# google-research/tnco

Hardware: AMD Instinct MI355X
Metric: SA move-evaluations/s (whole node) + best log10(flops) vs ref, 512-leaf TN (higher is better)
Workload: dtype f64

## Files before the change

tnco_amd/csrc/sa_sweep.h:

```cpp
#pragma once
#include "sa_kernels.h"
#include "fw_params.h"

#include <type_traits>

namespace tnco {

#define TNCO_LANDED(x) __asm__ volatile("" : "+v"(x) : : "memory")

#ifndef TNCO_NODE_ACCESS
#define TNCO_NODE_ACCESS 4
#endif

#define TNCO_LDS __attribute__((address_space(3)))
typedef TNCO_LDS volatile uint32_t lds_vu32;
typedef TNCO_LDS volatile int32_t lds_vi32;

__device__ __forceinline__ uint32_t mt_temper(uint32_t z) {
  z ^= (z >> 11);
  z ^= (z << 7) & 0x9d2c5680u;
  z ^= (z << 15) & 0xefc60000u;
  z ^= (z >> 18);
  return z;
}

constexpr int MT_SHADOW = 64;

constexpr int MT_ROUND_RING = 64;
constexpr int MT_ROUND_LOW = 8;
static_assert(MT_ROUND_RING <= MT_SHADOW && MT_ROUND_LOW >= 7, "refill rounds");

typedef uint32_t rng_u32x4 __attribute__((ext_vector_type(4)));
struct RngPcv { rng_u32x4 pcv; };
struct RngNoPcv {};
template <int LOG2L, int RINGX = 0, bool PCV = false>
struct Rng : std::conditional_t<PCV, RngPcv, RngNoPcv> {
  static constexpr int L = 1 << LOG2L;
  static constexpr int NL = L < 4 ? L : 4;
  static constexpr int SB = 4 * NL;
  static constexpr int RING = RINGX ? RINGX : ((2 * SB > 16) ? 2 * SB : 16);
  static_assert(RING <= MT_SHADOW && (RING & (RING - 1)) == 0 && RING >= 2 * SB, "ring size");

  struct __attribute__((packed, aligned(4))) U4 { uint32_t x[4]; };

  uint32_t* mt_base;
  uint32_t* sh_base;
  uint32_t r32;
  lds_vu32* ring;
  int lig;
  __device__ __forceinline__ uint32_t* st() const { return mt_base + (uint64_t)r32 * 624u; }
  __device__ __forceinline__ uint32_t* shadow() const { return sh_base + (uint64_t)r32 * (uint32_t)MT_SHADOW; }
  uint32_t cons, prod, tw;
  bool pend, ptw;
  typedef rng_u32x4 u32x4;
  u32x4 pa;
  uint32_t pb, pc[4];
  typedef u32x4 u32x4w __attribute__((aligned(4)));

  __device__ __forceinline__ uint32_t gen_of_cons() const { return cons == 0 ? 0u : (cons - 1u) / 624u; }

  __device__ __forceinline__ void request() {
    const uint32_t k0 = prod % 624u;
    ptw = prod >= tw;
    if (lig < NL) {
      const int k = (int)k0 + 4 * lig;
      const uint32_t* s = st();
      pa = *reinterpret_cast<const u32x4*>(s + k);
      if (ptw) {
        pb = s[(k + 4 == 624) ? 0 : k + 4];
        if (k == 224) {
          if constexpr (PCV) { this->pcv.x = s[621]; this->pcv.y = s[622]; this->pcv.z = s[623]; this->pcv.w = s[0]; }
          else { pc[0] = s[621]; pc[1] = s[622]; pc[2] = s[623]; pc[3] = s[0]; }
        } else {
          int km = k + 397;
          if (km >= 624) km -= 624;
          if constexpr (PCV) {
            this->pcv = *reinterpret_cast<const u32x4w*>(s + km);
          } else {
            const U4 c = *reinterpret_cast<const U4*>(s + km);
            pc[0] = c.x[0]; pc[1] = c.x[1]; pc[2] = c.x[2]; pc[3] = c.x[3];
          }
        }
      }
    }
    pend = true;
  }
  __device__ __forceinline__ void produce() {
    if (lig < NL) {
      const uint32_t nx[4] = {pa[1], pa[2], pa[3], pb};
      uint32_t v[4];
#pragma unroll
      for (int j = 0; j < 4; ++j) {
        v[j] = pa[j];
        if (ptw) {
          const uint32_t y = (pa[j] & 0x80000000u) | (nx[j] & 0x7fffffffu);
          uint32_t c;
          if constexpr (PCV) c = this->pcv[j]; else c = pc[j];
          v[j] = c ^ (y >> 1) ^ ((y & 1u) ? 0x9908b0dfu : 0u);
        }
        ring[(prod + (uint32_t)(4 * lig + j)) & (RING - 1)] = mt_temper(v[j]);
      }
      if (ptw) {
        const int sidx = (int)(prod % 624u) + 4 * lig;
        *reinterpret_cast<uint4*>(st() + sidx) = make_uint4(v[0], v[1], v[2], v[3]);
        if ((prod / 624u) > gen_of_cons())
          *reinterpret_cast<uint4*>(shadow() + sidx) = make_uint4(pa[0], pa[1], pa[2], pa[3]);
      }
    }
    if (ptw) tw = prod + SB;
    prod += SB;
    pend = false;
  }
  __device__ __forceinline__ bool room() const { return !pend && (prod - cons) + SB <= (uint32_t)RING; }

  template <int FILL = 0>
  __device__ __forceinline__ void init(const Params& P, int64_t r, lds_vu32* ring_, int mti, int mtw,
                                       int lig_) {
    mt_base = P.mt; sh_base = P.mtshadow; r32 = (uint32_t)r; ring = ring_; lig = lig_;
    pend = false; ptw = false;
    pb = 0;
    pa = (u32x4)(0u);
#pragma unroll
    for (int j = 0; j < 4; ++j) pc[j] = 0;
    if constexpr (PCV) this->pcv = (u32x4)(0u);
    if (mti >= 624) { cons = 624; tw = 624; } else { cons = (uint32_t)mti; tw = (uint32_t)mtw; }
    prod = cons & ~(uint32_t)(SB - 1);
    for (int b = 0; (FILL == 0 || b < FILL) && room(); ++b) {
      request();
      produce();
    }
  }
  __device__ __forceinline__ uint32_t next() {
    const uint32_t v = ring[cons & (RING - 1)];
    ++cons;
    return v;
  }
  __device__ __forceinline__ uint32_t next_sync() {
    if (cons == prod) {
      if (!pend) request();
      produce();
    }
    return next();
  }
  __device__ __forceinline__ void prefetch() {
    if (room()) request();
  }
  __device__ __forceinline__ uint32_t avail() const { return prod - cons; }
  __device__ __forceinline__ double uniform01() {
    const uint32_t x1 = next();
    const uint32_t x2 = next();
    double s = (double)x1 + (double)x2 * 4294967296.0;
    double r = s * 5.421010862427522170037e-20;
    if (r >= 1.0) r = 0.99999999999999988897769753748;
    return r;
  }
  __device__ __forceinline__ void finish(int& mti, int& mtw) {
    if (pend) produce();
    const uint32_t g = gen_of_cons();
    mti = (int)(cons - 624u * g);
    if (tw > 624u * (g + 1u)) {
      const uint32_t nw = tw - 624u * (g + 1u);
      for (uint32_t k = (uint32_t)lig; k < nw; k += L) st()[k] = shadow()[k];
      mtw = 624;
    } else {
      mtw = (int)(tw - 624u * g);
    }
  }
};

#ifndef TNCO_ACCEPT_PATH
#define TNCO_ACCEPT_PATH(p)
#endif

__device__ __attribute__((noinline)) bool accept_exact(double x, double beta, double u, int f32) {
  return u <= rnd_cost(pow(x, -beta), f32);
}

__device__ __forceinline__ bool accept_move(int kind, double beta, double delta, double total, double u,
                                            int f32) {
  if (kind == 0) { TNCO_ACCEPT_PATH(0); return true; }
  if (delta <= 0) { TNCO_ACCEPT_PATH(0); return true; }
  if (kind == 1) { TNCO_ACCEPT_PATH(1); return u <= 0.0; }
  if (total == 0) { TNCO_ACCEPT_PATH(1); return u <= 0.0; }
  const double x = rnd_cost(1.0 + rnd_cost(delta / total, f32), f32);
  const float uf = (float)u, xf = (float)x, bf = (float)beta;
  const float lu = __log2f(uf), lx = __log2f(xf);
  const float lp = -bf * lx;
  const float margin = (fabsf(lp) + fabsf(lu)) * 2e-6f + fabsf(bf) * 3e-7f + 1e-5f;
  if (uf > 1e-30f && xf < 1e30f && fabsf(lp) < 1e30f && beta >= 0.0) {
#ifdef TNCO_CHECK_ACCEPT
    if (lu < lp - margin || lu > lp + margin) {
      const bool fast = lu < lp - margin;
      if (fast != accept_exact(x, beta, u, f32)) __builtin_trap();
      return fast;
    }
#else
    if (lu < lp - margin) { TNCO_ACCEPT_PATH(2); return true; }
    if (lu > lp + margin) { TNCO_ACCEPT_PATH(3); return false; }
#endif
  }
  TNCO_ACCEPT_PATH(4);
  return accept_exact(x, beta, u, f32);
}

#ifndef TNCO_WAVES_PER_SIMD
#define TNCO_WAVES_PER_SIMD 3
#endif
enum : int { S_BEGIN = 0, S_GOT_B = 1, S_GOT_HB = 2, S_GOT_B1 = 3, S_GOT_HA = 4, S_MOVE = 5, S_END = 6 };

struct WalkScal {
  double total, beta, pP, pO, pC, raC, rnC;
  int raL, raR, raP, rnL, rnR, rnP, raW, rnW;
  uint32_t n_moves, n_acc;
};
struct ColdState {
  double min_cost;
  uint32_t jmin, n_impr, n_full, n_rpick;
};
typedef TNCO_LDS volatile ColdState lds_cold;

#ifdef TNCO_PROFILE
#define TNCO_PROF_DECL unsigned long long pt_[5] = {0, 0, 0, 0, 0}, pa_[5] = {0, 0, 0, 0, 0}
#if TNCO_PROFILE == 2
#define TNCO_PROF_T(i)                                           \
  do {                                                           \
    if ((i) == 1) pt_[0] = __builtin_amdgcn_s_memtime();         \
    if ((i) == 2) pt_[4] = __builtin_amdgcn_s_memtime();         \
  } while (0)
#define TNCO_PROF_F(i) pt_[i] = __builtin_amdgcn_s_memtime()
#else
#define TNCO_PROF_T(i) pt_[i] = __builtin_amdgcn_s_memtime()
#define TNCO_PROF_F(i)
#endif
#define TNCO_PROF_ACC                                            \
  do {                                                           \
    pa_[0] += pt_[1] - pt_[0]; pa_[1] += pt_[2] - pt_[1];        \
    pa_[2] += pt_[3] - pt_[2]; pa_[3] += pt_[4] - pt_[3];        \
    pa_[4] += 1;                                                 \
  } while (0)
#define TNCO_PROF_OUT(rs) \
  for (int k_ = 0; k_ < 5; ++k_) (rs)->pad1[k_] += pa_[k_]
#else
#define TNCO_PROF_DECL
#define TNCO_PROF_T(i)
#define TNCO_PROF_F(i)
#define TNCO_PROF_ACC
#define TNCO_PROF_OUT(rs)
#endif

#ifndef TNCO_SWEEP_THREADS
#define TNCO_SWEEP_THREADS 256
#endif
constexpr int SWT = TNCO_SWEEP_THREADS;
#ifndef TNCO_FW_STAGED_WAVES
#define TNCO_FW_STAGED_WAVES 2
#endif
#ifndef TNCO_LEAN_RULE
#define TNCO_LEAN_RULE (FW && !GENERIC && !HYPER && LOG2L == 2)
#endif
template <int LOG2L, int K, bool HYPER, bool GENERIC, bool FW = false, bool SPREAD = false>
#ifndef TNCO_HYPER_WAVES
#define TNCO_HYPER_WAVES 2
#endif
#ifndef TNCO_GENERIC_WAVES
#define TNCO_GENERIC_WAVES 2
#endif
#ifndef TNCO_K4_WAVES
#define TNCO_K4_WAVES 2
#endif
__device__ __forceinline__ void sa_run_body(
    const Params& P, const double* __restrict__ betas, const int64_t n_steps, const int prob_kind,
    const FwParams& F, const int tail_last, const int block0) {
  constexpr int L = 1 << LOG2L;
  constexpr int GPB = SWT >> LOG2L;
  using M = Mask<K>;
  constexpr bool ROUNDS = !HYPER && !GENERIC && !FW;
  constexpr bool RPCV = ROUNDS && TNCO_NODE_ACCESS >= 4;
  using R = Rng<LOG2L, ROUNDS ? MT_ROUND_RING : 0, RPCV>;
  static_assert(!ROUNDS || R::SB + 1 >= MT_ROUND_LOW, "refill rounds: the prologue");
  __shared__ uint32_t rngbuf[GPB * R::RING];
  __shared__ ColdState coldbuf[GPB];
  __shared__ int32_t jbuf[GPB * 16];
  constexpr bool LEAN = TNCO_LEAN_RULE;
  __shared__ WalkScal scalbuf[LEAN ? GPB : 1];
  __shared__ uint64_t slbuf[LEAN && FW ? GPB * L * K : 1];
  __shared__ double tabbuf[GENERIC ? (L * K * 64 + 1) : 1];
  __shared__ uint64_t clsbuf[GENERIC ? (TABS_MAXCLS * L * K) : 1];
  __shared__ uint64_t oddbuf[GENERIC ? (L * K) : 1];
  if constexpr (GENERIC) {
    const bool use_ctab = P.cost_mode == 1 || (P.cost_mode == 2 && P.odd_single);
    if (use_ctab) {
      for (int i = threadIdx.x; i < P.W * 64 + 1; i += SWT) tabbuf[i] = P.ctab[i];
    } else if (P.cost_mode == 2) {
      for (int i = threadIdx.x; i < L * K * 64; i += SWT) tabbuf[i] = P.dimsd[i];
    }
    if (P.cost_mode >= 2) {
      for (int i = threadIdx.x; i < P.n_dimclass * L * K; i += SWT) clsbuf[i] = P.dimclass[i];
      if (P.cost_mode == 2)
        for (int i = threadIdx.x; i < L * K; i += SWT) oddbuf[i] = P.oddmask[i];
    }
    __syncthreads();
  }

  const int tid = threadIdx.x;
  const int lig = tid & (L - 1);
  const int gbase = (tid & 63) & ~(L - 1);
  const int seats = SPREAD ? block0 : (64 >> LOG2L);
  const int gw = (tid & 63) >> LOG2L;
  const bool master = !SPREAD || gw < seats;
  const int seat = SPREAD ? (gw & (seats - 1)) : gw;
  const int gib = SPREAD ? (tid >> 6) * (64 >> LOG2L) + seat : tid >> LOG2L;
  const int64_t r = SPREAD ? ((int64_t)blockIdx.x * (SWT / 64) + (tid >> 6)) * seats + seat
                           : ((int64_t)blockIdx.x + block0) * GPB + gib;
  if (r >= P.R || n_steps <= 0) return;
  const bool lane0 = (lig == 0) && master;
  const int slig = master ? lig : (1 << 20);

  const int n = P.n, N = P.N;
  constexpr bool HYD = HYPER;
  constexpr bool CP = !HYPER && !GENERIC && !FW;
  constexpr bool QHDR = CP && TNCO_NODE_ACCESS >= 1, PAIRS = CP && TNCO_NODE_ACCESS >= 2, PSEL = CP && TNCO_NODE_ACCESS >= 3 && LPS == 1;
  View<LOG2L, K, HYPER, !FW, PAIRS> v;
  v.init(P, P.blocks + r * P.RB, nullptr, lig);
  auto lpar = [&]() -> int32_t* { return P.lpar + r * (int64_t)n * LPS; };
  lds_cold& cold = *((lds_cold*)coldbuf + gib);

  R rng;
  {
    const ReplicaState* rs = P.rs + r;
    rng.template init<ROUNDS ? 2 : 0>(P, r, (lds_vu32*)rngbuf + gib * R::RING, rs->mti, rs->mtw, master ? lig : 64);
    if (lane0) {
      cold.min_cost = rs->min_cost;
      cold.jmin = rs->jmin;
      cold.n_impr = 0; cold.n_full = 0; cold.n_rpick = 0;
    }
  }
  const uint32_t jcap = (uint32_t)P.jcap;
  uint32_t jtail = P.rs[r].jtail;
  bool jinvalid = P.rs[r].jinvalid != 0;
  auto jb = [&](int i) -> lds_vi32& { return *((lds_vi32*)jbuf + gib * 16 + i); };
  auto jlog = [&]() -> int32_t* {
    uint32_t rr = rng.r32;
    __asm__ volatile("" : "+v"(rr));
    return P.jlog + (int64_t)rr * (int64_t)P.jcap;
  };
  if ((jtail & 15u) != 0u) {
    for (int q = slig; q < 4; q += L) {
      const int4 t = *reinterpret_cast<const int4*>(jlog() + (jtail & ~15u) + 4 * q);
      jb(4 * q + 0) = t.x; jb(4 * q + 1) = t.y; jb(4 * q + 2) = t.z; jb(4 * q + 3) = t.w;
    }
  }
  M sl_regs = mzero<K>();
  typedef TNCO_LDS volatile uint64_t lds_vu64;
  [[maybe_unused]] lds_vu64* slw = (lds_vu64*)slbuf + (LEAN && FW ? gib * (L * K) : 0);
  [[maybe_unused]] bool impr_any = false;
  if constexpr (FW) {
    const uint64_t* s0 = F.slices + r * 2 * (int64_t)(L * K);
#pragma unroll
    for (int k = 0; k < K; ++k) {
      if constexpr (LEAN && FW) slw[v.widx(k)] = s0[v.widx(k)]; else sl_regs.w[k] = s0[v.widx(k)];
    }
  }
  [[maybe_unused]] TabsLds<K> tabs{P, (lds_cdouble*)tabbuf, (lds_cu64*)clsbuf, (lds_cu64*)oddbuf, mzero<K>()};
  if constexpr (GENERIC) {
    if (P.sparse != nullptr) {
#pragma unroll
      for (int k = 0; k < K; ++k) tabs.sp.w[k] = P.sparse[k * L + lig];
    }
  }
  const int f32 = GENERIC ? P.f32 : 0;
  const int log2d = P.log2d;
  const bool disable_shared = P.disable_shared != 0;
  const int nsteps32 = (int)n_steps;

  int B = 0, bl = 0, br = 0, A = -1;
  [[maybe_unused]] int wB = 0;
  double ccB = 0, partB = 0;
  WalkScal scal_regs{0, 0, 0, 0, 0, 0, 0, -1, -1, -1, -1, -1, -1, 0, 0, 0, 0};
  TNCO_LDS volatile WalkScal* scal_lds = (TNCO_LDS volatile WalkScal*)scalbuf + (LEAN ? gib : 0);
  auto& S = *[&]() {
    if constexpr (LEAN) return scal_lds; else return &scal_regs;
  }();
  if constexpr (CP) {
    double t0 = P.rs[r].total;
    TNCO_LANDED(t0);
    S.total = t0;
  }
  if constexpr (LEAN) {
    S.total = 0; S.beta = 0; S.pP = 0; S.pO = 0; S.pC = 0; S.raC = 0; S.rnC = 0;
    S.raL = -1; S.raR = -1; S.raP = -1; S.rnL = -1; S.rnR = -1; S.rnP = -1; S.raW = 0; S.rnW = 0; S.n_moves = 0; S.n_acc = 0;
  }
  M mP = mzero<K>(), mO = mzero<K>(), hB = mzero<K>();
  bool pl = true;
  M mC = mzero<K>(), hA = mzero<K>();
  int step = 0;
  int state = S_BEGIN;

  int stC = 0, stE = 0;
  [[maybe_unused]] double stW64 = 0;
  [[maybe_unused]] double stQ0 = 0, stQ1 = 0;
  int x_al = 0, x_ar = 0, x_aP = -1;
  double x_ccA = 0, x_partA = 0, x_pCcur = 0;
  int gL = -1, gR = -1, gP = -1;
  [[maybe_unused]] int gW = 0;
  double gC = 0;
  [[maybe_unused]] double gQ1 = 0;
  typedef int32_t i32x4 __attribute__((ext_vector_type(4)));
  [[maybe_unused]] i32x4 gLRP = (i32x4)(-1);
  [[maybe_unused]] u32x2 gHq = (u32x2)(0u);
  M gM = mzero<K>(), gH = mzero<K>();
  [[maybe_unused]] PairStage<K> gMq;
  if constexpr (PAIRS) {
#pragma unroll
    for (int j = 0; j < (K / 2 ? K / 2 : 1); ++j) gMq.p[j] = (u64x2)(0ull);
    gMq.s = 0ull;
  }
  uint32_t gXlo = 0, gXhi = 0;

  TNCO_PROF_DECL;
  for (;;) {
    TNCO_PROF_T(0);
    if (rng.pend) rng.produce();
    TNCO_PROF_T(1);

    bool acc = false, did_move = false, did_end = false, improved = false;

    if (state == S_END) {
      did_end = true;
      const bool close_sweep = !FW || tail_last != 0 || step != nsteps32 - 1;
      if constexpr (CP) {
        stQ0 = pl ? S.pP : S.pO;
        stQ1 = pl ? S.pO : S.pP;
      }
      if (close_sweep && partB < cold.min_cost) {
        if constexpr (FW) impr_any = true;
        if (lane0) {
          cold.min_cost = partB;
          cold.n_impr = cold.n_impr + 1;
        }
        if (jinvalid) {
          if (lane0) {
            NodeRec o;
            o.left = bl; o.right = br; o.parent = -1; o.pad = 0; o.ccost = CP ? stQ0 : ccB; o.partial = CP ? stQ1 : partB;
            *v.hdr(B) = o;
          }
          v.lpar = lpar();
          Links* __restrict__ ml = P.minlinks + r * (int64_t)N;
          for (int i0 = slig; i0 < N; i0 += 4 * L) {
            int4 h4[4];
#pragma unroll
            for (int q = 0; q < 4; ++q) {
              const int i = i0 + q * L;
              h4[q] = make_int4(-1, -1, -1, 0);
              if (i < n) h4[q].z = v.lpar[(int64_t)i * LPS];
              else if (i < N) h4[q] = *reinterpret_cast<const int4*>(v.hdr(i));
            }
#pragma unroll
            for (int q = 0; q < 4; ++q) {
              const int i = i0 + q * L;
              if (i < N) {
                Links o;
                o.left = h4[q].x; o.right = h4[q].y; o.parent = h4[q].z; o.pad = 0;
                ml[i] = o;
              }
            }
          }
          jtail = 0;
          jinvalid = false;
          if (lane0) cold.n_full = cold.n_full + 1;
        }
        improved = true;
      }
      if constexpr (CP) S.total = partB;
      ++step;
      state = (step >= nsteps32) ? -1 : S_BEGIN;
    }

    TNCO_PROF_F(1);
    int hN = -1, x1 = -1, yN = -1;
    const uint32_t* xa = nullptr;
    if (state == S_BEGIN) {
      const uint32_t x = rng.next();
      x_al = (int)(x % (uint32_t)n);
      x1 = x_al;
      xa = reinterpret_cast<const uint32_t*>(lpar() + (int64_t)x_al * LPS);
    } else if (state == S_GOT_B) {
      hN = B;
      if constexpr (CP) x1 = B;
      else xa = reinterpret_cast<const uint32_t*>(&v.hdr(B)->partial);
    } else if (CP && state == S_GOT_HB) {
      xa = reinterpret_cast<const uint32_t*>(betas + step);
      if (A >= 0) {
        hN = A;
        x1 = A;
      }
    } else if (state == S_GOT_HB) {
      x1 = pl ? br : bl;
      hN = A;
      yN = B;
      xa = reinterpret_cast<const uint32_t*>(&v.hdr(N - 1)->partial);
    } else if (state == S_GOT_B1) {
      xa = reinterpret_cast<const uint32_t*>(betas + step);
      if (A >= 0) {
        hN = S.raP;
        yN = A;
        x1 = (S.raL == B) ? S.raR : S.raL;
      }
    } else if (state == S_MOVE) {
      if constexpr (CP) {
        if (S.raP >= 0) {
          hN = S.raP;
          x1 = S.raP;
        }
      } else if (S.raP >= 0) {
        x1 = (S.rnL == A) ? S.rnR : S.rnL;
        hN = S.rnP;
        yN = S.raP;
      }
    }

    TNCO_PROF_F(2);
    if constexpr (QHDR) {
      int lq = lig;
      __asm__ volatile("" : "+v"(lq));
      v.lig = lq;
    }
    if (hN >= 0) {
      const NodeRec* q = v.hdr(hN);
      if constexpr (QHDR) {
        gHq = *reinterpret_cast<const u32x2*>(v.blk + v.hdr_piece_off(hN));
      } else {
        if constexpr (CP) gLRP = *reinterpret_cast<const i32x4*>(q);
        else { gL = q->left; gR = q->right; gP = q->parent; }
        gC = q->ccost;
        if constexpr (FW) gW = q->pad;
        if constexpr (CP) gQ1 = q->pright;
      }
    }
    double gMp = 0;
    if (x1 >= 0) {
      if constexpr (PAIRS) v.pair_stage_into(gMq, x1);
      else v.mask_stage_into(gM, x1);
      if constexpr (!CP)
        if (x1 >= n) gMp = v.hdr(x1)->partial;
    }
    if (xa != nullptr) {
      gXlo = xa[0];
      gXhi = xa[1];
    }
    if constexpr (HYPER) {
      if (yN >= 0) v.mask_stage_into(gH, yN);
    }
    if constexpr (ROUNDS) {
      const bool need = !rng.pend && rng.avail() < (uint32_t)MT_ROUND_LOW;
      const bool round = __ballot(need) != 0;
      if (round && rng.room()) rng.request();
    } else {
      if (rng.room()) rng.request();
    }
    TNCO_PROF_F(3);

    if (state == S_MOVE) {
      did_move = true;
      int al = S.raL, ar = S.raR;
      const int aP = S.raP;
      double ccA = S.raC;
      const bool c_is_right = (al == B);
      const int C = c_is_right ? ar : al;

      const M hy = HYD ? mand<K>(hB, mor<K>(mand<K>(hA, mC), mand<K>(mP, mO))) : mzero<K>();
      M sl = sl_regs;
      if constexpr (LEAN && FW) {
#pragma unroll
        for (int k = 0; k < K; ++k) sl.w[k] = slw[v.widx(k)];
      }
      constexpr bool PICK_FIRST = !GENERIC && FW;
      bool interP, interO;
      int pcAP = 0, pcBP = 0, pcAO = 0, pcBO = 0;
      if constexpr (!GENERIC && !PICK_FIRST) {
        uint32_t wP = mpopc<K>(mor<K>(mor<K>(mor<K>(mxor<K>(mP, mC), hy), mO), sl)) |
                      (mpopc<K>(mor<K>(mor<K>(mP, mC), sl)) << 13) | ((mnonzero<K>(mand<K>(mP, mC)) ? 1u : 0u) << 26);
        uint32_t wO = mpopc<K>(mor<K>(mor<K>(mor<K>(mxor<K>(mO, mC), hy), mP), sl)) |
                      (mpopc<K>(mor<K>(mor<K>(mO, mC), sl)) << 13) | ((mnonzero<K>(mand<K>(mO, mC)) ? 1u : 0u) << 26);
        wP = gsum<LOG2L>(wP);
        wO = gsum<LOG2L>(wO);
        interP = (wP >> 26) != 0;
        interO = (wO >> 26) != 0;
        pcAP = (int)(wP & 0x1fffu); pcBP = (int)((wP >> 13) & 0x1fffu);
        pcAO = (int)(wO & 0x1fffu); pcBO = (int)((wO >> 13) & 0x1fffu);
      } else {
        const uint32_t w = gsum<LOG2L>((mnonzero<K>(mand<K>(mP, mC)) ? 1u : 0u) |
                                       ((mnonzero<K>(mand<K>(mO, mC)) ? 1u : 0u) << 8));
        interP = (w & 0xffu) != 0;
        interO = (w >> 8) != 0;
      }
      bool pick0;
      if (disable_shared || (interP && interO)) {
        pick0 = (rng.next() & 1u) != 0;
        if (lane0) cold.n_rpick = cold.n_rpick + 1;
      } else {
        pick0 = pl ? interP : interO;
      }
      const bool pickP = pick0 == pl;
      const M mD = msel<K>(pickP, mP, mO), mE = msel<K>(pickP, mO, mP);
      const M newB = mor<K>(mxor<K>(mD, mC), hy);
      const double pD = pickP ? S.pP : S.pO, pE = pickP ? S.pO : S.pP;
      const int E = pick0 ? br : bl;
      if constexpr (PICK_FIRST) {
        const uint32_t w = gsum<LOG2L>(mpopc<K>(mor<K>(mor<K>(newB, mE), sl)) | (mpopc<K>(mor<K>(mor<K>(mD, mC), sl)) << 13));
        pcAP = pcAO = (int)(w & 0x1fffu);
        pcBP = pcBO = (int)((w >> 13) & 0x1fffu);
      }

      [[maybe_unused]] double new_width_B = 0;
      bool fits = true;
      if constexpr (FW) {
        double sliced_width;
        if constexpr (!GENERIC) {
          const uint32_t x = gsum<LOG2L>(mpopc<K>(newB) | (mpopc<K>(mandn<K>(newB, sl)) << 16));
          new_width_B = (double)(log2d * (int)(x & 0xffffu));
          sliced_width = (double)(log2d * (int)(x >> 16));
        } else if (F.log2dims == nullptr && P.sparse == nullptr) {
          const uint32_t x = gsum<LOG2L>(mpopc<K>(newB) | (mpopc<K>(mandn<K>(newB, sl)) << 16));
          new_width_B = fw_wr(F, F.log2d * (double)(x & 0xffffu));
          sliced_width = fw_wr(F, F.log2d * (double)(x >> 16));
        } else {
          new_width_B = fw_width<LOG2L, K>(P, F, newB, lig, gbase);
          sliced_width = fw_width<LOG2L, K>(P, F, mandn<K>(newB, sl), lig, gbase);
        }
        fits = sliced_width <= F.max_width;
      }
      double nA, nB;
      if constexpr (!GENERIC) {
        nA = pow2_cost(log2d * (pickP ? pcAP : pcAO), 0);
        nB = pow2_cost(log2d * (pickP ? pcBP : pcBO), 0);
      } else {
        nA = generic_cost_t<LOG2L, K>(P, tabs, mor<K>(mor<K>(newB, mE), sl), lig, gbase);
        nB = generic_cost_t<LOG2L, K>(P, tabs, mor<K>(mor<K>(mD, mC), sl), lig, gbase);
      }
      const double delta = rnd_cost(rnd_cost(nB - ccB, f32) + rnd_cost(nA - ccA, f32), f32);
      ++S.n_moves;

      if (fits) {
        const double u = rng.uniform01();
        acc = accept_move(prob_kind, S.beta, delta, S.total, u, f32);
      }

      double pEcur = pE, pCcur = S.pC;
      M mBnow, mX;
      stC = C; stE = E;
      if (acc) {
        ++S.n_acc;
        if constexpr (FW) {
          if (F.width_f32) wB = __float_as_int((float)new_width_B);
          stW64 = new_width_B;
        }
        if (pick0) br = C; else bl = C;
        if (c_is_right) ar = E; else al = E;
        if constexpr (HYD) hB = newB;
        ccB = nB;
        ccA = nA;
        S.total = rnd_cost(S.total + delta, f32);
        pEcur = S.pC;
        pCcur = pE;
        mBnow = newB;
        mX = mE;
      } else {
        mBnow = HYD ? hB : mxor<K>(mP, mO);
        mX = mC;
      }
      if constexpr (CP) {
        stQ0 = pick0 ? pD : pEcur;
        stQ1 = pick0 ? pEcur : pD;
      }
      partB = rnd_cost(rnd_cost(pD + pEcur, f32) + ccB, f32);
      const double partA = rnd_cost(rnd_cost(partB + pCcur, f32) + ccA, f32);
      x_al = al; x_ar = ar; x_aP = aP; x_ccA = ccA; x_partA = partA; x_pCcur = pCcur;
      mP = mBnow; mO = mX; pl = c_is_right;
    }

    TNCO_PROF_T(2);
    if constexpr (QHDR) {
      TNCO_LANDED(gHq);
    } else {
      TNCO_LANDED(gL); TNCO_LANDED(gR); TNCO_LANDED(gP); TNCO_LANDED(gC);
      if constexpr (CP) { TNCO_LANDED(gQ1); TNCO_LANDED(gLRP); }
    }
    if constexpr (FW) TNCO_LANDED(gW);
    TNCO_LANDED(gMp); TNCO_LANDED(gXlo); TNCO_LANDED(gXhi);
    if constexpr (PAIRS) {
#pragma unroll
      for (int j = 0; j < K / 2; ++j) TNCO_LANDED(gMq.p[j]);
      if constexpr (K & 1) TNCO_LANDED(gMq.s);
    } else {
#pragma unroll
      for (int k = 0; k < K; ++k) {
        TNCO_LANDED(gM.w[k]);
        if constexpr (HYPER) { TNCO_LANDED(gH.w[k]); }
      }
    }
    TNCO_LANDED(rng.pb);
    TNCO_LANDED(rng.pa);
#pragma unroll
    for (int j = 0; j < 4; ++j) TNCO_LANDED(rng.pc[j]);
    if constexpr (RPCV) TNCO_LANDED(rng.pcv);

    TNCO_PROF_T(3);
    if constexpr (QHDR) {
      int lq = lig;
      __asm__ volatile("" : "+v"(lq));
      v.lig = lq;
    }
    if (did_move && acc) {
      if (!jinvalid) {
        if (jtail == jcap) {
          jinvalid = true;
        } else {
          if (lane0) jb((int)(jtail & 15u)) = stE;
          ++jtail;
          if ((jtail & 15u) == 0u) {
            for (int q = slig; q < 4; q += L)
              *reinterpret_cast<int4*>(jlog() + (jtail - 16u) + 4 * q) =
                  make_int4(jb(4 * q + 0), jb(4 * q + 1), jb(4 * q + 2), jb(4 * q + 3));
          }
        }
      }
      v.lpar = lpar();
      if (master) {
        if constexpr (PSEL) {
          v.set_parent_lane0(stC, B);
          v.set_parent_lane0(stE, A);
        } else {
          v.set_parent_group(stC, B);
          v.set_parent_group(stE, A);
        }
        if constexpr (PAIRS) v.set_mask_pairs(B, mP);
        else v.set_mask(B, mP);
      }
    }
    if (did_move || did_end) {
      if constexpr (QHDR) {
        if (master && v.lig < 4) {
          const uint64_t q0 = __double_as_longlong(stQ0), q1 = __double_as_longlong(stQ1);
          u32x2 o;
          const int lq = v.lig;
          o.x = lq == 0 ? (uint32_t)bl : (lq == 1 ? (uint32_t)A : (uint32_t)(lq == 2 ? q0 : q1));
          o.y = lq == 0 ? (uint32_t)br : (lq == 1 ? 0u : (uint32_t)((lq == 2 ? q0 : q1) >> 32));
          *reinterpret_cast<u32x2*>(v.blk + v.hdr_piece_off(B)) = o;
        }
      } else if (lane0) {
        NodeRec o;
        o.left = bl; o.right = br; o.parent = A; o.pad = FW ? wB : 0;
        if constexpr (CP) { o.pleft = stQ0; o.pright = stQ1; } else { o.ccost = ccB; o.partial = partB; }
        *v.hdr(B) = o;
        if constexpr (FW) {
          if (did_move && acc && !F.width_f32) F.width64[(int64_t)rng.r32 * N + B] = stW64;
        }
      }
#ifdef TNCO_FIRST64
      if (!(did_move && acc))
        v.set_mask_first(B, did_move ? mP : (HYD ? hB : mxor<K>(mP, mO)));
#endif
      if (improved && lane0) cold.jmin = jtail;
      if (state < 0) break;
    }
    TNCO_PROF_T(4);
    TNCO_PROF_ACC;

    if constexpr (QHDR) {
      gL = (int)quad_bcast<0>(gHq.x); gR = (int)quad_bcast<0>(gHq.y); gP = (int)quad_bcast<1>(gHq.x);
      gC = __hiloint2double((int)quad_bcast<2>(gHq.y), (int)quad_bcast<2>(gHq.x));
      gQ1 = __hiloint2double((int)quad_bcast<3>(gHq.y), (int)quad_bcast<3>(gHq.x));
    } else if constexpr (CP) { gL = gLRP.x; gR = gLRP.y; gP = gLRP.z; }
    if constexpr (PAIRS) gM = v.pair_landed(gMq);
    auto land_A = [&]() {
      S.raL = gL; S.raR = gR; S.raP = gP;
      const M mB = mxor<K>(mP, mO);
      mC = mxor<K>(gM, mB);
      S.pC = (gL == B) ? gQ1 : gC;
      S.raC = pow2_cost(log2d * (int)gsum<LOG2L>(mpopc<K>(mor<K>(mB, gM))), 0);
    };
    if (CP && did_move) {
      S.pP = partB; S.pO = x_pCcur;
      B = A; bl = x_al; br = x_ar; ccB = x_ccA; partB = x_partA;
      A = x_aP;
      if (A >= 0) land_A();
      state = (A < 0) ? S_END : S_MOVE;
    } else if (CP && state == S_GOT_B) {
      bl = gL; br = gR; A = gP;
      pl = gL == x_al;
      mO = mxor<K>(gM, mP);
      S.pO = pl ? gQ1 : gC;
      partB = S.total;
      ccB = pow2_cost(log2d * (int)gsum<LOG2L>(mpopc<K>(mor<K>(mP, mO))), 0);
      state = S_GOT_HB;
    } else if (CP && state == S_GOT_HB) {
      S.beta = __hiloint2double((int)gXhi, (int)gXlo);
      if (A >= 0) land_A();
      state = (A < 0) ? S_END : S_MOVE;
    } else if (did_move) {
      S.pP = partB; S.pO = x_pCcur;
      B = A; bl = x_al; br = x_ar; ccB = x_ccA; partB = x_partA;
      if constexpr (HYPER) { hB = hA; hA = gH; }
      A = x_aP;
      S.raL = S.rnL; S.raR = S.rnR; S.raP = S.rnP; S.raC = S.rnC;
      S.rnL = gL; S.rnR = gR; S.rnP = gP; S.rnC = gC;
      if constexpr (FW) { wB = S.raW; S.raW = S.rnW; S.rnW = gW; }
      mC = gM;
      S.pC = gMp;
      state = (A < 0) ? S_END : S_MOVE;
    } else if (state == S_BEGIN) {
      B = (int)gXlo;
      mP = gM; S.pP = CP ? 0.0 : gMp;
      state = S_GOT_B;
    } else if (state == S_GOT_B) {
      bl = gL; br = gR; A = gP; ccB = gC;
      if constexpr (FW) wB = gW;
      partB = __hiloint2double((int)gXhi, (int)gXlo);
      pl = gL == x_al;
      state = S_GOT_HB;
    } else if (state == S_GOT_HB) {
      mO = gM; S.pO = gMp;
      S.total = __hiloint2double((int)gXhi, (int)gXlo);
      S.raL = gL; S.raR = gR; S.raP = gP; S.raC = gC;
      if constexpr (FW) S.raW = gW;
      if constexpr (HYPER) { hB = gH; }
      state = S_GOT_B1;
    } else if (state == S_GOT_B1) {
      mC = gM; S.pC = gMp;
      S.beta = __hiloint2double((int)gXhi, (int)gXlo);
      S.rnL = gL; S.rnR = gR; S.rnP = gP; S.rnC = gC;
      if constexpr (FW) S.rnW = gW;
      if constexpr (HYPER) { hA = gH; }
      state = (A < 0) ? S_END : S_MOVE;
    }
  }

  if ((jtail & 15u) != 0u) {
    for (int q = slig; q < 4; q += L)
      *reinterpret_cast<int4*>(jlog() + (jtail & ~15u) + 4 * q) =
          make_int4(jb(4 * q + 0), jb(4 * q + 1), jb(4 * q + 2), jb(4 * q + 3));
  }
  if constexpr (FW) {
    if (impr_any) {
      uint64_t* s1 = F.slices + r * 2 * (int64_t)(L * K) + L * K;
#pragma unroll
      for (int k = 0; k < K; ++k)
        if (master) s1[v.widx(k)] = (LEAN && FW) ? (uint64_t)slw[v.widx(k)] : sl_regs.w[k];
    }
  }
  int mti, mtw;
  rng.finish(mti, mtw);
  if (lane0) {
    ReplicaState* rs = P.rs + r;
    if constexpr (CP) rs->total = S.total;
    rs->jmin = cold.jmin; rs->jtail = jtail;
    rs->jinvalid = jinvalid ? 1 : 0;
    rs->n_fullcopy += cold.n_full;
    rs->min_cost = cold.min_cost;
    rs->n_moves += S.n_moves;
    rs->n_accepted += S.n_acc;
    rs->n_improved += cold.n_impr;
    rs->n_randpick += cold.n_rpick;
    rs->mti = mti;
    rs->mtw = mtw;
    if constexpr (!FW) { TNCO_PROF_OUT(rs); }
  }
}

template <int LOG2L, int K, bool HYPER, bool GENERIC, bool FW = false, bool SPREAD = false>
__global__ __launch_bounds__(SWT, (LOG2L == 1 ? 2 : (FW ? TNCO_FW_STAGED_WAVES : (HYPER ? TNCO_HYPER_WAVES : (GENERIC ? TNCO_GENERIC_WAVES : (K >= 4 ? TNCO_K4_WAVES : TNCO_WAVES_PER_SIMD)))))) void sa_run_kernel(
    const Params P, const double* __restrict__ betas, const int64_t n_steps, const int prob_kind,
    const FwParams F, const int tail_last, const int block0) {
  sa_run_body<LOG2L, K, HYPER, GENERIC, FW, SPREAD>(P, betas, n_steps, prob_kind, F, tail_last, block0);
}

template <int LOG2L, int K, bool SPREAD = false>
__global__ __launch_bounds__(SWT, 2) __attribute__((amdgpu_num_vgpr(96))) void sa_run_fw_kernel(
    const Params P, const double* __restrict__ betas, const int64_t n_steps, const int prob_kind,
    const FwParams F, const int tail_last, const int block0) {
  sa_run_body<LOG2L, K, false, false, true, SPREAD>(P, betas, n_steps, prob_kind, F, tail_last, block0);
}
template <int LOG2L, int K, bool HYPER, bool GENERIC, bool SPREAD>
__host__ inline auto fw_staged_kernel() {
  if constexpr (!HYPER && !GENERIC && LOG2L == 2) return &sa_run_fw_kernel<LOG2L, K, SPREAD>;
  else return &sa_run_kernel<LOG2L, K, HYPER, GENERIC, true, SPREAD>;
}

}
```

Measured before the change: 10.58 billion.

## Stream move state advance into move phase and unify landing with branchless selects

Adds a TNCO_MOVE_STREAM mode, default 2, for the CP+QHDR path. It advances the walk state (B, A, bl, br, ccB, partB) inside the move step and stages the header record and store targets (stB, stA, stRec). The landing phase becomes one branch-light block that computes the popcount cost once for all states. It also enables PICK_FIRST for CP and offers an optional predicated-select accept path (level 3). The aim is to shorten the serial dependency chain and cut divergent control flow per SA step, at the cost of extra live registers and more complex state bookkeeping.

```diff
diff --git a/tnco_amd/csrc/sa_sweep.h b/tnco_amd/csrc/sa_sweep.h
--- a/tnco_amd/csrc/sa_sweep.h
+++ b/tnco_amd/csrc/sa_sweep.h
@@ -10,6 +10,10 @@
 
 #ifndef TNCO_NODE_ACCESS
 #define TNCO_NODE_ACCESS 4
+#endif
+
+#ifndef TNCO_MOVE_STREAM
+#define TNCO_MOVE_STREAM 2
 #endif
 
 #define TNCO_LDS __attribute__((address_space(3)))
@@ -399,6 +403,16 @@
   int stC = 0, stE = 0;
   [[maybe_unused]] double stW64 = 0;
   [[maybe_unused]] double stQ0 = 0, stQ1 = 0;
+  constexpr bool MS2 = CP && QHDR && TNCO_MOVE_STREAM >= 2, MS3 = CP && TNCO_MOVE_STREAM >= 3;
+  [[maybe_unused]] int stB = 0, stA = -1;
+  [[maybe_unused]] u32x2 stRec = (u32x2)(0u);
+  auto rec_piece = [&](int lq, int l, int r_, int p, double q0d, double q1d) -> u32x2 {
+    const uint64_t q0 = __double_as_longlong(q0d), q1 = __double_as_longlong(q1d);
+    u32x2 o;
+    o.x = lq == 0 ? (uint32_t)l : (lq == 1 ? (uint32_t)p : (uint32_t)(lq == 2 ? q0 : q1));
+    o.y = lq == 0 ? (uint32_t)r_ : (lq == 1 ? 0u : (uint32_t)((lq == 2 ? q0 : q1) >> 32));
+    return o;
+  };
   int x_al = 0, x_ar = 0, x_aP = -1;
   double x_ccA = 0, x_partA = 0, x_pCcur = 0;
   int gL = -1, gR = -1, gP = -1;
@@ -472,6 +486,7 @@
         improved = true;
       }
       if constexpr (CP) S.total = partB;
+      if constexpr (MS2) { stB = B; stA = -1; }
       ++step;
       state = (step >= nsteps32) ? -1 : S_BEGIN;
     }
@@ -525,6 +540,9 @@
       __asm__ volatile("" : "+v"(lq));
       v.lig = lq;
     }
+    if constexpr (MS2) {
+      if (did_end) stRec = rec_piece(v.lig & 3, bl, br, -1, stQ0, stQ1);
+    }
     if (hN >= 0) {
       const NodeRec* q = v.hdr(hN);
       if constexpr (QHDR) {
@@ -574,7 +592,7 @@
 #pragma unroll
         for (int k = 0; k < K; ++k) sl.w[k] = slw[v.widx(k)];
       }
-      constexpr bool PICK_FIRST = !GENERIC && FW;
+      constexpr bool PICK_FIRST = !GENERIC && (FW || (CP && TNCO_MOVE_STREAM >= 1));
       bool interP, interO;
       int pcAP = 0, pcBP = 0, pcAO = 0, pcBO = 0;
       if constexpr (!GENERIC && !PICK_FIRST) {
@@ -649,7 +667,20 @@
       double pEcur = pE, pCcur = S.pC;
       M mBnow, mX;
       stC = C; stE = E;
-      if (acc) {
+      if constexpr (MS3) {
+        S.n_acc += acc ? 1u : 0u;
+        br = (acc && pick0) ? C : br;
+        bl = (acc && !pick0) ? C : bl;
+        ar = (acc && c_is_right) ? E : ar;
+        al = (acc && !c_is_right) ? E : al;
+        ccB = acc ? nB : ccB;
+        ccA = acc ? nA : ccA;
+        S.total = acc ? rnd_cost(S.total + delta, f32) : S.total;
+        pEcur = acc ? S.pC : pE;
+        pCcur = acc ? pE : S.pC;
+        mBnow = mxor<K>(mD, msel<K>(acc, mC, mE));
+        mX = msel<K>(acc, mE, mC);
+      } else if (acc) {
         ++S.n_acc;
         if constexpr (FW) {
           if (F.width_f32) wB = __float_as_int((float)new_width_B);
@@ -675,7 +706,15 @@
       }
       partB = rnd_cost(rnd_cost(pD + pEcur, f32) + ccB, f32);
       const double partA = rnd_cost(rnd_cost(partB + pCcur, f32) + ccA, f32);
-      x_al = al; x_ar = ar; x_aP = aP; x_ccA = ccA; x_partA = partA; x_pCcur = pCcur;
+      if constexpr (MS2) {
+        stB = B; stA = A;
+        stRec = rec_piece(v.lig & 3, bl, br, A, stQ0, stQ1);
+        S.pP = partB; S.pO = pCcur;
+        B = A; bl = al; br = ar; ccB = ccA; partB = partA;
+        A = aP;
+      } else {
+        x_al = al; x_ar = ar; x_aP = aP; x_ccA = ccA; x_partA = partA; x_pCcur = pCcur;
+      }
       mP = mBnow; mO = mX; pl = c_is_right;
     }
 
@@ -726,28 +765,25 @@
         }
       }
       v.lpar = lpar();
+      const int sB = MS2 ? stB : B, sA = MS2 ? stA : A;
       if (master) {
         if constexpr (PSEL) {
-          v.set_parent_lane0(stC, B);
-          v.set_parent_lane0(stE, A);
+          v.set_parent_lane0(stC, sB);
+          v.set_parent_lane0(stE, sA);
         } else {
-          v.set_parent_group(stC, B);
-          v.set_parent_group(stE, A);
+          v.set_parent_group(stC, sB);
+          v.set_parent_group(stE, sA);
         }
-        if constexpr (PAIRS) v.set_mask_pairs(B, mP);
-        else v.set_mask(B, mP);
+        if constexpr (PAIRS) v.set_mask_pairs(sB, mP);
+        else v.set_mask(sB, mP);
       }
     }
     if (did_move || did_end) {
-      if constexpr (QHDR) {
-        if (master && v.lig < 4) {
-          const uint64_t q0 = __double_as_longlong(stQ0), q1 = __double_as_longlong(stQ1);
-          u32x2 o;
-          const int lq = v.lig;
-          o.x = lq == 0 ? (uint32_t)bl : (lq == 1 ? (uint32_t)A : (uint32_t)(lq == 2 ? q0 : q1));
-          o.y = lq == 0 ? (uint32_t)br : (lq == 1 ? 0u : (uint32_t)((lq == 2 ? q0 : q1) >> 32));
-          *reinterpret_cast<u32x2*>(v.blk + v.hdr_piece_off(B)) = o;
-        }
+      if constexpr (MS2) {
+        if (master && v.lig < 4) *reinterpret_cast<u32x2*>(v.blk + v.hdr_piece_off(stB)) = stRec;
+      } else if constexpr (QHDR) {
+        if (master && v.lig < 4)
+          *reinterpret_cast<u32x2*>(v.blk + v.hdr_piece_off(B)) = rec_piece(v.lig, bl, br, A, stQ0, stQ1);
       } else if (lane0) {
         NodeRec o;
         o.left = bl; o.right = br; o.parent = A; o.pad = FW ? wB : 0;
@@ -759,7 +795,7 @@
       }
 #ifdef TNCO_FIRST64
       if (!(did_move && acc))
-        v.set_mask_first(B, did_move ? mP : (HYD ? hB : mxor<K>(mP, mO)));
+        v.set_mask_first(MS2 ? stB : B, did_move ? mP : (HYD ? hB : mxor<K>(mP, mO)));
 #endif
       if (improved && lane0) cold.jmin = jtail;
       if (state < 0) break;
@@ -780,7 +816,32 @@
       S.pC = (gL == B) ? gQ1 : gC;
       S.raC = pow2_cost(log2d * (int)gsum<LOG2L>(mpopc<K>(mor<K>(mB, gM))), 0);
     };
-    if (CP && did_move) {
+    if constexpr (MS2) {
+      const bool in_begin = !did_move && state == S_BEGIN, in_b = !did_move && state == S_GOT_B;
+      const bool in_a = did_move || (!in_begin && !in_b);
+      if (in_begin) {
+        B = (int)gXlo;
+        mP = gM; S.pP = 0.0;
+      }
+      if (!did_move && state == S_GOT_HB) S.beta = __hiloint2double((int)gXhi, (int)gXlo);
+      const bool land = in_a && A >= 0;
+      const double cc = pow2_cost(log2d * (int)gsum<LOG2L>(mpopc<K>(mor<K>(msel<K>(in_b, mP, mxor<K>(mP, mO)), gM))), 0);
+      if (land) {
+        S.raL = gL; S.raR = gR; S.raP = gP;
+        mC = mxor<K>(gM, mxor<K>(mP, mO));
+        S.pC = (gL == B) ? gQ1 : gC;
+        S.raC = cc;
+      }
+      if (in_b) {
+        bl = gL; br = gR; A = gP;
+        pl = gL == x_al;
+        mO = mxor<K>(gM, mP);
+        S.pO = pl ? gQ1 : gC;
+        partB = S.total;
+        ccB = cc;
+      }
+      state = in_begin ? S_GOT_B : (in_b ? S_GOT_HB : (A < 0 ? S_END : S_MOVE));
+    } else if (CP && did_move) {
       S.pP = partB; S.pO = x_pCcur;
       B = A; bl = x_al; br = x_ar; ccB = x_ccA; partB = x_partA;
       A = x_aP;
```

Measured after the change: 10.59 billion, median of 6. No clear change (+0.2%).
